# irfanfadhullah/unet_zoo

Measured on AMD Instinct MI355X. Metric: images/sec (fwd+bwd) at B=16 3x256x256, 1/2/4/8 MI355X, higher is better.
Workload: dtype bf16; 1 GPU; unet train step (zero_grad+fwd+BCE+bwd+clip+AdamW), B=16/GPU 3x256x256, random-init weights; global_batch=16, parallelism=dp1

## Files before the change

include/unetzoo_hip.h:

```cpp
#ifndef UNETZOO_HIP_H
#define UNETZOO_HIP_H

#include <stddef.h>
#include <stdint.h>

#ifdef __cplusplus
extern "C" {
#endif

#define UZ_ABI_VERSION 1

enum { UZ_F32 = 0, UZ_BF16 = 1 };

enum {
  UZ_OK = 0,
  UZ_EINVAL = -1,
  UZ_ENOTIMPL = -2
};

enum {
  UZ_TAPS_CONV = 0,
  UZ_TAPS_GATHER2X2 = 1,
  UZ_TAPS_CONV_UP2 = 2,
  UZ_TAPS_CONV_S2 = 3
// ... 10 lines not shown
int uz_build_ablate(void);
const char* uz_source_hash(void);
int uz_clock_probe(int iters, void* out_pairs, int workgroups, void* stream);
int uz_set_cu_reserve(int n);
int uz_get_cu_reserve(void);

typedef struct uz_conv_desc {
  int dtype;
  int N, H, W;
  int Hin, Win;
  int Cin, ldx;
  int Nout, ldy;
  int ntaps, taps_mode, dil;
  int store_mode, Co;
  int Hout, Wout;
} uz_conv_desc;

int uz_conv_igemm_grid_m(const uz_conv_desc* d);
int uz_conv_igemm_kernel_name(const uz_conv_desc* d, int with_workspace, char* buf, int cap);
int uz_conv_igemm(const uz_conv_desc* d, const void* x, const void* w_packed, const float* bias,
                  void* y, float* stats_partial, void* stream);
int uz_conv_igemm_res(const uz_conv_desc* d, const void* x, const void* w_packed, const float* bias,
                      const void* res, int ldres, void* y, void* stream);
int uz_conv_igemm_res_ws(const uz_conv_desc* d, const void* x, const void* w_packed, const float* bias,
                         const void* res, int ldres, void* y, void* workspace, void* stream);
long long uz_conv_igemm_workspace_bytes(const uz_conv_desc* d);
int uz_conv_igemm_ws_grid_m(const uz_conv_desc* d);
int uz_conv_igemm_ws(const uz_conv_desc* d, const void* x, const void* w_packed, const float* bias,
                     void* y, float* stats_partial, void* workspace, void* stream);
int uz_conv_igemm_bnred_supported(const uz_conv_desc* d);
int uz_conv_igemm_bnred(const uz_conv_desc* d, const void* x, const void* w_packed, void* y, const void* bn_y,
                        int ld_bny, const float* scale, const float* shift, const float* mean, const float* invstd,
                        float* partial, void* stream);

int uz_conv_igemm_xf_supported(const uz_conv_desc* d);
int uz_conv_igemm_xf(const uz_conv_desc* d, const void* x, const float* in_scale, const float* in_shift,
                     const void* w_packed, const float* bias, void* y, float* stats_partial, void* stream);

int uz_conv_igemm_bnact_supported(const uz_conv_desc* d);
int uz_conv_igemm_bnact(const uz_conv_desc* d, const void* x, const void* w_packed, const float* bias,
                        const float* out_scale, const float* out_shift, int relu, void* y, void* stream);

typedef struct uz_wgrad_desc {
  int dtype;
  int N, H, W;
  int Hr, Wr;
  int Ci, ldl;
  int Cj, ldr;
  int ntaps, taps_mode, dil;
} uz_wgrad_desc;

int uz_wgrad_split(const uz_wgrad_desc* d);
long long uz_wgrad_workspace_bytes(const uz_wgrad_desc* d);
int uz_wgrad(const uz_wgrad_desc* d, const void* L, const void* R, float* out, void* workspace,
             void* stream);
int uz_wgrad_kernel_name(const uz_wgrad_desc* d, char* buf, int cap);
int uz_wgrad_xf_supported(const uz_wgrad_desc* d);
int uz_wgrad_xf(const uz_wgrad_desc* d, const void* L, const void* R, const float* r_scale, const float* r_shift,
                float* out, void* workspace, void* stream, int phase);
int uz_wgrad_phase(const uz_wgrad_desc* d, const void* L, const void* R, float* out, void* workspace, void* stream,
                   int phase);
typedef struct {
  uz_wgrad_desc desc;
  const void* L;
  const void* R;
  float* out;
// ... 383 lines not shown
```

unet_zoo_amd/_lib.py:

```python
from __future__ import annotations

import ctypes
import os
from ctypes import POINTER, Structure, c_char_p, c_double, c_float, c_int, c_void_p

import torch

UZ_F32, UZ_BF16 = 0, 1
TAPS_CONV, TAPS_GATHER2X2, TAPS_CONV_UP2, TAPS_CONV_S2 = 0, 1, 2, 3
STORE_PLAIN, STORE_SHUFFLE2X2 = 0, 1
PACK_CONV_FWD, PACK_CONV_DGRAD, PACK_CONVT_FWD, PACK_CONVT_DGRAD, PACK_IM2COL, PACK_VEC_REPEAT = range(6)

LIB_NAME = "libunetzoo_hip.so"
LIB_PATH = os.environ.get("UNET_ZOO_AMD_LIB") or os.path.join(os.path.dirname(os.path.abspath(__file__)), LIB_NAME)

EXPORTS = (
    "uz_abi_version", "uz_last_error_string", "uz_build_ablate", "uz_source_hash", "uz_set_cu_reserve", "uz_get_cu_reserve", "uz_clock_probe", "uz_conv_igemm_grid_m", "uz_conv_igemm",
    "uz_wgrad_split", "uz_wgrad_workspace_bytes", "uz_wgrad", "uz_wgrad_kernel_name", "uz_wgrad_phase", "uz_wgrad_xf_supported", "uz_wgrad_xf", "uz_conv3x3_first_supported", "uz_conv3x3_first_rows", "uz_conv3x3_first_fwd",
    "uz_conv3x3_first_wgrad_workspace_bytes", "uz_conv3x3_first_wgrad", "uz_conv3x3_first_wgrad_bn", "uz_pack_weights", "uz_pack_weights_batched", "uz_pack_conv3x3_batched", "uz_im2col3x3_nchw", "uz_bn_finalize",
    "uz_bn_eval_scale", "uz_bn_relu_apply", "uz_bn_relu_bwd_workspace_bytes", "uz_bn_relu_bwd_reduce", "uz_bn_relu_bwd_apply",
    "uz_outconv_fwd", "uz_outconv_fwd_xf", "uz_outconv_bwd_workspace_bytes", "uz_outconv_bwd", "uz_outconv_bwd_rows", "uz_outconv_bwd_bnred", "uz_bn_relu_bwd_apply_head_supported", "uz_bn_relu_bwd_apply_head",
    "uz_colsum",
    "uz_attn_grid", "uz_attn_psi_fwd", "uz_attn_gate_fwd", "uz_attn_bwd_psi", "uz_attn_bwd_reduce",
    "uz_attn_bwd_apply", "uz_sum_rows", "uz_sum_rows_f32", "uz_sum2x2",
    "uz_bn_relu_add_apply", "uz_bn_relu_add_apply_fin", "uz_bn_relu_bwd_reduce_rows", "uz_bn_relu_bwd_apply_fin", "uz_bilinear_fwd", "uz_bilinear_bwd", "uz_resize_bilinear_fwd", "uz_resize_bilinear_bwd", "uz_resample2",
    "uz_pool_grad_combine",
    "uz_sideconv3x3_fwd", "uz_sideconv3x3_bwd_workspace_bytes", "uz_sideconv3x3_bwd",
    "uz_fuse1x1_fwd", "uz_fuse1x1_bwd_workspace_bytes", "uz_fuse1x1_bwd",
    "uz_conv_igemm_workspace_bytes", "uz_conv_igemm_ws_grid_m", "uz_conv_igemm_ws",
    "uz_conv_igemm_bnred_supported", "uz_conv_igemm_bnred", "uz_conv_igemm_xf_supported", "uz_conv_igemm_xf", "uz_conv_igemm_kernel_name", "uz_bn_bwd_finalize", "uz_profile_arm", "uz_profile_disarm",
    "uz_patchify", "uz_layernorm_fwd", "uz_layernorm_bwd_rows", "uz_layernorm_bwd", "uz_layernorm_act_bwd",
    "uz_ln_head_fwd", "uz_ln_head_bwd_workspace_bytes", "uz_ln_head_bwd", "uz_sum_rows_f32_ld",
    "uz_winattn_fwd", "uz_winattn_bwd_rows", "uz_winattn_bwd",
    "uz_colsum_workspace_bytes", "uz_colsum_ws", "uz_colstats_rows", "uz_colstats", "uz_cpb_fwd", "uz_cpb_bwd",
    "uz_cpb_fwd_batched", "uz_cpb_bwd_batched_workspace_bytes", "uz_cpb_bwd_batched",
    "uz_clip_adamw_workspace_bytes", "uz_clip_adamw",
    "uz_gelu_fwd", "uz_gelu_bwd", "uz_dwconv3x3", "uz_dwconv3x3_wgrad_rows", "uz_dwconv3x3_wgrad",
    "uz_space_to_depth", "uz_space_to_depth_crop", "uz_im2col_nchw", "uz_sra_fwd", "uz_sra_bwd_workspace_bytes", "uz_sra_bwd",
    "uz_bce_dice_workspace_bytes", "uz_bce_dice", "uz_colsum_batched_workspace_bytes", "uz_colsum_batched", "uz_sum_rows_f32_batched", "uz_conv_igemm_res", "uz_wgrad_multi_workspace_bytes", "uz_wgrad_multi", "uz_conv_igemm_res_ws",
    "uz_add_relu", "uz_relu_bwd", "uz_pil_resample_h_u8", "uz_pil_resample_v_f32",
    "uz_gemm_nt", "uz_softmax_fwd", "uz_softmax_bwd", "uz_adaptive_avgpool_fwd", "uz_adaptive_avgpool_bwd",
    "uz_rowdot_f32", "uz_cast_rows", "uz_wgrad_batched_workspace_bytes", "uz_wgrad_batched", "uz_wgrad_batched2",
    "uz_softmax_workspace_bytes", "uz_add_map", "uz_dropout", "uz_chanscale_relu", "uz_chanattn_probs_fwd", "uz_chanattn_probs_bwd",
    "uz_conv5x5_grid_m", "uz_conv5x5", "uz_wgrad5x5_workspace_bytes", "uz_wgrad5x5",
    "uz_bn_elu_apply", "uz_bn_elu_bwd_rows", "uz_bn_elu_bwd_reduce", "uz_bn_elu_bwd_apply",
    "uz_conv_igemm_bnact_supported", "uz_conv_igemm_bnact", "uz_conv3x3_first_fwd_bnact",
    "uz_region_loss_workspace_bytes", "uz_region_loss",
)


class ConvDesc(Structure):
    _fields_ = [(n, c_int) for n in (
        "dtype", "N", "H", "W", "Hin", "Win", "Cin", "ldx", "Nout", "ldy", "ntaps", "taps_mode",
        "dil", "store_mode", "Co", "Hout", "Wout")]


class WgradDesc(Structure):
    _fields_ = [(n, c_int) for n in (
        "dtype", "N", "H", "W", "Hr", "Wr", "Ci", "ldl", "Cj", "ldr", "ntaps", "taps_mode", "dil")]


class Conv5Desc(Structure):
    _fields_ = [(n, c_int) for n in ("dtype", "N", "H", "W", "Cin", "ldx", "Nout", "ldy", "ksize")]


class Wgrad5Desc(Structure):
    _fields_ = [(n, c_int) for n in ("dtype", "N", "H", "W", "Ci", "ldl", "Cj", "ldr", "ksize", "CiOut", "CjOut")]


class BnEluBwdDesc(Structure):
    _fields_ = [(n, c_int) for n in ("dtype", "N", "HW", "C", "ldx", "ldo", "ldg0", "ldg1", "ldg2", "lddx", "ldgres", "flags")]


class BnBwdDesc(Structure):
    _fields_ = [(n, c_int) for n in (
        "dtype", "N", "H", "W", "C", "ldy", "ldg0", "ldg1", "ldgp", "lddy", "pool_ceil")]


class LnDesc(Structure):
    _fields_ = [(n, c_int) for n in ("dtype", "N", "Ho", "Wo", "C", "ldx", "ldy", "ldr", "ldg", "lddx", "mode", "r")] \
        + [("eps", c_float), ("act", c_int)]


class WinAttnDesc(Structure):
    _fields_ = [(n, c_int) for n in ("dtype", "B", "H", "W", "C", "heads", "ws", "shift", "Nt", "ldq", "ldo")] \
        + [("scale", c_float)]

# ... 65 lines not shown
    global _lib
    if _lib is not None:
        return _lib
    if not os.path.exists(LIB_PATH):
        raise HipLibraryError(
            f"{LIB_PATH} not found: the HIP kernel library is not built. Run "
            "`python -c 'import __graft_entry__ as g; g.build()'` from the repo root. "
            "unet_zoo_amd has no CPU fallback.")
    lib = ctypes.CDLL(LIB_PATH)
    lib.uz_abi_version.restype = c_int
    lib.uz_last_error_string.restype = c_char_p
    lib.uz_source_hash.restype = c_char_p
    lib.uz_source_hash.argtypes = []
    vp, ip, fp = c_void_p, c_int, c_float
    lib.uz_set_cu_reserve.argtypes = [c_int]
    lib.uz_clock_probe.argtypes = [c_int, vp, c_int, vp]
    lib.uz_get_cu_reserve.argtypes = []
    lib.uz_conv_igemm_grid_m.argtypes = [POINTER(ConvDesc)]
    lib.uz_conv_igemm.argtypes = [POINTER(ConvDesc), vp, vp, vp, vp, vp, vp]
    lib.uz_conv_igemm_res.argtypes = [POINTER(ConvDesc), vp, vp, vp, vp, ip, vp, vp]
    lib.uz_conv_igemm_res_ws.argtypes = [POINTER(ConvDesc), vp, vp, vp, vp, ip, vp, vp, vp]
    lib.uz_conv_igemm_workspace_bytes.argtypes = [POINTER(ConvDesc)]
    lib.uz_conv_igemm_ws_grid_m.argtypes = [POINTER(ConvDesc)]
    lib.uz_conv_igemm_ws.argtypes = [POINTER(ConvDesc), vp, vp, vp, vp, vp, vp, vp]
    lib.uz_conv_igemm_bnred_supported.argtypes = [POINTER(ConvDesc)]
    lib.uz_conv_igemm_xf_supported.argtypes = [POINTER(ConvDesc)]
    lib.uz_conv_igemm_xf.argtypes = [POINTER(ConvDesc), vp, vp, vp, vp, vp, vp, vp, vp]
    lib.uz_conv_igemm_bnact_supported.argtypes = [POINTER(ConvDesc)]
    lib.uz_conv_igemm_bnact.argtypes = [POINTER(ConvDesc), vp, vp, vp, vp, vp, c_int, vp, vp]
    lib.uz_conv_igemm_kernel_name.argtypes = [POINTER(ConvDesc), c_int, c_char_p, c_int]
    lib.uz_profile_arm.argtypes = [vp, vp]
    lib.uz_profile_disarm.argtypes = []
    lib.uz_conv_igemm_bnred.argtypes = [POINTER(ConvDesc), vp, vp, vp, vp, c_int, vp, vp, vp, vp, vp, vp]
    lib.uz_bn_bwd_finalize.argtypes = [vp, c_int, c_int, vp, vp, vp, vp]
    lib.uz_patchify.argtypes = [ip, vp, ip, ip, ip, ip, ip, ip, vp, vp]
    lib.uz_layernorm_fwd.argtypes = [POINTER(LnDesc), vp, vp, vp, vp, vp, vp, vp, vp]
    lib.uz_layernorm_act_bwd.argtypes = [POINTER(LnDesc), vp, vp, vp, vp, vp, vp, vp, vp]
    lib.uz_layernorm_bwd_rows.argtypes = [POINTER(LnDesc)]
    lib.uz_layernorm_bwd.argtypes = [POINTER(LnDesc), vp, vp, vp, vp, vp, vp, vp, vp]
    lib.uz_ln_head_fwd.argtypes = [POINTER(LnDesc), vp, vp, vp, vp, vp, ip, vp, vp, vp]
    lib.uz_ln_head_bwd_workspace_bytes.argtypes = [POINTER(LnDesc), ip]
    lib.uz_ln_head_bwd.argtypes = [POINTER(LnDesc), vp, vp, vp, vp, ip, vp, vp, vp, vp, vp, vp, vp, vp, vp]
    lib.uz_sum_rows_f32_ld.argtypes = [vp, ip, ip, ip, vp, ip, vp, vp]
    lib.uz_winattn_fwd.argtypes = [POINTER(WinAttnDesc), vp, vp, vp, vp, vp, vp]
    lib.uz_winattn_bwd_rows.argtypes = [POINTER(WinAttnDesc)]
    lib.uz_winattn_bwd.argtypes = [POINTER(WinAttnDesc), vp, vp, vp, vp, vp, vp, ip, vp, ip, vp, vp]
    lib.uz_colstats_rows.argtypes = [ip, ip, ip]
    lib.uz_colstats.argtypes = [ip, vp, ip, ip, ip, vp, vp]
    lib.uz_cpb_fwd.argtypes = [vp, vp, vp, vp, vp, ip, ip, ip, vp, vp]
    lib.uz_cpb_bwd.argtypes = [vp, vp, vp, vp, vp, ip, ip, ip, vp, vp, vp, vp, vp]
    lib.uz_cpb_fwd_batched.argtypes = [vp, ip, vp]
    lib.uz_cpb_bwd_batched_workspace_bytes.argtypes = [vp, ip]
    lib.uz_cpb_bwd_batched.argtypes = [vp, ip, vp, vp]
    lib.uz_clip_adamw_workspace_bytes.argtypes = []
    lib.uz_clip_adamw.argtypes = [vp, vp, vp, vp, ctypes.c_longlong, fp, fp, fp, fp, fp, fp, vp, vp, vp]
    lib.uz_wgrad_split.argtypes = [POINTER(WgradDesc)]
    lib.uz_wgrad_workspace_bytes.argtypes = [POINTER(WgradDesc)]
    lib.uz_wgrad.argtypes = [POINTER(WgradDesc), vp, vp, vp, vp, vp]
    lib.uz_wgrad_kernel_name.argtypes = [POINTER(WgradDesc), c_char_p, c_int]
    lib.uz_wgrad_phase.argtypes = [POINTER(WgradDesc), vp, vp, vp, vp, vp, c_int]
    lib.uz_wgrad_xf_supported.argtypes = [POINTER(WgradDesc)]
    lib.uz_wgrad_xf.argtypes = [POINTER(WgradDesc), vp, vp, vp, vp, vp, vp, vp, c_int]
    lib.uz_conv3x3_first_supported.argtypes = [ip, ip, ip]
    lib.uz_conv3x3_first_rows.argtypes = [ip, ip, ip]
    lib.uz_conv3x3_first_fwd.argtypes = [ip, vp, ip, ip, ip, ip, vp, vp, ip, vp, ip, vp, vp]
    lib.uz_conv3x3_first_fwd_bnact.argtypes = [ip, vp, ip, ip, ip, ip, vp, vp, ip, vp, vp, ip, vp, ip, vp]
# ... 191 lines not shown
```

unet_zoo_amd/engine.py:

```python
from __future__ import annotations

import math
from typing import Callable, Dict, List, Optional, Sequence, Tuple

import torch
import torch.nn as nn

from . import _lib as L
from . import ops
from .ops import Act


def _round_up(a: int, b: int) -> int:
    return (a + b - 1) // b * b


class PackCache:

    def __init__(self):
        self.entries: Dict[tuple, tuple] = {}
        self._table: Optional[torch.Tensor] = None
        self._total = 0
        self._n = 0
        self._table_dtype = None
# ... 59 lines not shown
        begin = 0
        for i, (p, mode, kpad, dst) in enumerate(generic):
            if mode == L.PACK_VEC_REPEAT:
                arr[i] = L.PackItem(p.data_ptr(), dst.data_ptr(), begin, mode, p.numel(), 1, kpad, 0, 0)
                begin += dst.numel()
                continue
            d0, d1 = p.shape[0], p.shape[1]
            T = p.numel() // (d0 * d1)
            co, ci = (d0, d1) if mode in (L.PACK_CONV_FWD, L.PACK_CONV_DGRAD, L.PACK_IM2COL) else (d1, d0)
            arr[i] = L.PackItem(p.data_ptr(), dst.data_ptr(), begin, mode, co, ci, T, kpad, 0)
            begin += dst.numel()
        self._table = torch.frombuffer(bytearray(bytes(arr)), dtype=torch.uint8).to(dev)
        self._total, self._n, self._table_dtype = begin, len(generic), dtype

class ImageInput:

    __slots__ = ("nchw", "kpad", "dtype", "_patches", "N", "H", "W")

    def __init__(self, nchw: torch.Tensor, kpad: int, dtype: torch.dtype):
        self.nchw, self.kpad, self.dtype, self._patches = nchw, kpad, dtype, None
        self.N, _, self.H, self.W = nchw.shape

    def patches(self) -> Act:
        if self._patches is None:
            self._patches = ops.im2col3x3_nchw(self.nchw, self.kpad, self.dtype)
        return self._patches


class Engine:
    direct_first_conv = True
    defer_linear_wgrads = True
    fuse_bn_reduce = True
    fuse_bn_reduce_convt = True
    fold_bn_apply = True
    fold_bn_apply_head = True
    fold_head_grad = True
    fold_first_bn_bwd = True
    fuse_bn_finalize = False
    FIN_FLAGS = 4096
    reverse_element_passes = True
    fold_bn_eval = False

    def __init__(self, dtype: torch.dtype, device: torch.device, training: bool, record: bool,
                 grad_sink: Optional[Callable[[nn.Parameter, torch.Tensor], None]] = None,
                 pack_cache: Optional[PackCache] = None, grads_in_place: bool = False,
                 fold_bn_eval: Optional[bool] = None):
        if fold_bn_eval is not None:
            self.fold_bn_eval = bool(fold_bn_eval)
        self.folded_layers = 0
        self.unfolded_layers = 0
        self.dtype = dtype
        self.device = device
        self.training = training
        self.record = record
        self.tape: List[Callable[[], None]] = []
        self.param_grads: Dict[nn.Parameter, torch.Tensor] = {}
        self.grad_sink = grad_sink
        self.bk = 64 if dtype == torch.bfloat16 else 32
        self._bn_channels = 0
        self._sums: Optional[torch.Tensor] = None
        self._sums_used = 0
        self._cache = pack_cache if pack_cache is not None else PackCache()
        self.grads_in_place = grads_in_place
        self._heads: List[Tuple[Callable[..., None], int]] = []
        self.grad_log: List[Tuple[int, nn.Parameter]] = []
        self._pending_colsums: List[Tuple[int, nn.Parameter, Act]] = []
# ... 565 lines not shown
        return out

    def input_nhwc(self, x: torch.Tensor, cpad: int = 8) -> Act:
        L.require_cuda(x)
        N, C, H, W = x.shape
        a = self.new_act(N, H, W, _round_up(C, cpad), needs_grad=False)
        a.buf.zero_()
        a.buf.view(N, H, W, a.C)[..., :C].copy_(x.permute(0, 2, 3, 1))
        return a

    def act_to_logits(self, x: Act, K: int) -> torch.Tensor:
        assert K <= x.C
        logits = x.buf.view(x.N, x.H, x.W, x.ld)[..., x.off:x.off + K].permute(0, 3, 1, 2).float().contiguous()
        if self.record:
            def bwd(g_logits: torch.Tensor):
                g = self.new_act(x.N, x.H, x.W, x.C)
                g.buf.zero_()
                g.buf.view(x.N, x.H, x.W, x.C)[..., :K].copy_(g_logits.permute(0, 2, 3, 1))
                x.add_grad(g)

            self._heads.append((bwd, 1))
        return logits

    def conv_transpose2x2(self, x: Act, m: nn.ConvTranspose2d, out: Act, sole_reader: bool = False) -> Act:
        assert m.kernel_size == (2, 2) and m.stride == (2, 2) and m.in_channels == x.C
        Co = m.out_channels
        assert out.C == Co and out.H - 2 * x.H in (0, 1) and out.W - 2 * x.W in (0, 1)
        if (out.H, out.W) != (2 * x.H, 2 * x.W):
            v = out.buf.view(out.N, out.H, out.W, out.ld)[..., out.off:out.off + Co]
            v[:, 2 * x.H:, :, :] = 0
            v[:, :, 2 * x.W:, :] = 0
        wp = self._pack(m.weight, L.PACK_CONVT_FWD)
        bias4 = self._cache.get(m.bias, L.PACK_VEC_REPEAT, 4, self.dtype) if m.bias is not None else None
        ops.conv_igemm(x, wp, bias4, out, ntaps=1, store_mode=L.STORE_SHUFFLE2X2, nout=4 * Co, co=Co)

        if self.record:
            def bwd():
                g = self._sum_grads(out, 1)[0]
                if m.bias is not None:
                    cs = g.channel_sums(out=self._dst(m.bias))
                    self._give_grad(m.bias, cs if cs is not None else ops.colsum(g, out=self._dst(m.bias)))
                self._give_grad(m.weight, ops.wgrad(x, g, tuple(m.weight.shape), ntaps=4,
                                                    taps_mode=L.TAPS_GATHER2X2, out=self._dst(m.weight)))
                if x.needs_grad:
                    dx = self.new_act(x.N, x.H, x.W, x.C)
                    src = getattr(x, "bn_src", None) if (sole_reader and self.fuse_bn_reduce_convt) else None
                    part = ops.conv_igemm(g, self._pack(m.weight, L.PACK_CONVT_DGRAD), None, dx, ntaps=4,
                                          taps_mode=L.TAPS_GATHER2X2, bnred=src)
                    if src is not None and part is not None:
                        dx.bn_partials = part
                    x.add_grad(dx)

            self.tape.append(bwd)
        return out

    def _total_grad(self, a: Act) -> Optional[Act]:
        gs = list(a.grads)
        if not gs:
            return None
        while len(gs) > 1:
            g1, g0 = gs.pop(), gs.pop()
            tot = self.new_act(a.N, a.H, a.W, a.C)
            ops.pool_grad_combine(a, g0, g1, None, tot)
            gs.append(tot)
        return gs[0]

    def linear(self, x: Act, lin: nn.Linear, out: Optional[Act] = None, residual: Optional[Act] = None) -> Act:
        assert lin.in_features == x.C
        y = out if out is not None else self.new_act(x.N, x.H, x.W, lin.out_features)
        ops.conv_igemm(x, self._pack(lin.weight, L.PACK_CONV_FWD), lin.bias.detach() if lin.bias is not None else None,
                       y, ntaps=1, res=residual)
        if self.record:
            def bwd():
                g = self._total_grad(y)
                if g is None:
                    return
                if residual is not None and residual.needs_grad:
                    residual.add_grad(g)
                if lin.bias is not None:
                    self._bias_grad(lin.bias, g)
                self._linear_wgrad(lin.weight, g, x)
# ... 1151 lines not shown
```

unet_zoo_amd/ops.py:

```python
from __future__ import annotations

from ctypes import byref
from typing import List, Optional, Sequence

import math

import torch

from . import _lib as L


class Act:

    __slots__ = ("buf", "off", "C", "N", "H", "W", "grads", "parts", "rparts", "needs_grad", "colsums", "bn_src",
                 "bn_partials", "lazy")

    def __init__(self, buf: torch.Tensor, off: int, C: int, N: int, H: int, W: int,
                 needs_grad: bool = True):
        assert buf.dim() == 2 and buf.is_contiguous() and buf.shape[0] == N * H * W
        assert 0 <= off and off + C <= buf.shape[1]
        self.buf, self.off, self.C, self.N, self.H, self.W = buf, off, C, N, H, W
        self.grads: List["Act"] = []
        self.parts: Optional[Sequence["Act"]] = None
        self.rparts: Optional[Sequence[tuple]] = None
# ... 288 lines not shown
            L.check(lib.uz_conv_igemm_xf(byref(d), x.ptr(), xform[0].data_ptr(), xform[1].data_ptr(), w_packed.data_ptr(),
                                         _p(bias), y.ptr(), _p(stats), L.stream_ptr()), "uz_conv_igemm_xf")
        return stats
    if bnred is not None:
        assert bias is None and res is None and not want_stats
        bn_y, vec4 = bnred
        if not lib.uz_conv_igemm_bnred_supported(byref(d)) or (bn_y.P, bn_y.C) != (y.P, y.C):
            bnred = None
        else:
            gm = L.check_count(lib.uz_conv_igemm_grid_m(byref(d)), "uz_conv_igemm_grid_m")
            part = torch.empty((gm, 2, d.Nout), dtype=torch.float32, device=x.buf.device)
            with _Timed(kname + "_bnred", 2.0 * M * d.Nout * K, es * (x.P * x.C + 2 * M * d.Nout + d.Nout * K)):
                L.check(lib.uz_conv_igemm_bnred(byref(d), x.ptr(), w_packed.data_ptr(), y.ptr(), bn_y.ptr(), bn_y.ld,
                                                vec4[0].data_ptr(), vec4[1].data_ptr(), vec4[2].data_ptr(),
                                                vec4[3].data_ptr(), part.data_ptr(), L.stream_ptr()),
                        "uz_conv_igemm_bnred")
            return part
    if res is not None:
        assert (res.P, res.C) == (y.P, y.C) and res.dtype == y.dtype and not want_stats
        if kname.startswith("gemm_dma") and store_mode == L.STORE_PLAIN:
            with _Timed(kname, 2.0 * M * d.Nout * K, es * (x.P * x.C + 2 * M * d.Nout + d.Nout * K)):
                L.check(lib.uz_conv_igemm_res_ws(byref(d), x.ptr(), w_packed.data_ptr(), _p(bias), res.ptr(), res.ld, y.ptr(),
                                                 _p(ws), L.stream_ptr()), "uz_conv_igemm_res_ws")
            return None
    with _Timed(kname, 2.0 * M * d.Nout * K,
                        es * (x.P * x.C + M * d.Nout + d.Nout * K)):
        L.check(lib.uz_conv_igemm_ws(byref(d), x.ptr(), w_packed.data_ptr(), _p(bias), y.ptr(), _p(stats),
                                     _p(ws), L.stream_ptr()), "uz_conv_igemm_ws")
    if res is not None:
        add_acts(y, res, y)
    return stats


def _bnact_desc(x: Act, nout: int, ldy: int, ntaps: int, dil: int, taps_mode: int):
    H, W = (2 * x.H, 2 * x.W) if taps_mode == L.TAPS_CONV_UP2 else (x.H, x.W)
    return L.ConvDesc(L.dtype_code(x.dtype), x.N, H, W, x.H, x.W, x.C, x.ld, nout, ldy, ntaps, taps_mode, dil,
                      L.STORE_PLAIN, 0, 0, 0)


def conv_bnact_supported(x: Act, nout: int, ldy: int, *, ntaps: int, dil: int = 1, taps_mode: int = L.TAPS_CONV) -> bool:
    if taps_mode not in (L.TAPS_CONV, L.TAPS_CONV_UP2):
        return False
    d = _bnact_desc(x, nout, ldy, ntaps, dil, taps_mode)
    return bool(L.load().uz_conv_igemm_bnact_supported(byref(d)))


def conv_igemm_bnact(x: Act, w_packed: torch.Tensor, bias: Optional[torch.Tensor], scale: torch.Tensor, shift: torch.Tensor,
                     relu: bool, y: Act, *, ntaps: int, dil: int = 1, taps_mode: int = L.TAPS_CONV) -> None:
    L.require_cuda(x.buf, w_packed, y.buf, scale, shift)
    d = _bnact_desc(x, y.C, y.ld, ntaps, dil, taps_mode)
    assert w_packed.dtype == x.dtype and y.dtype == x.dtype and (y.N, y.H, y.W) == (d.N, d.H, d.W)
    assert w_packed.shape == (d.Nout, ntaps * x.C), (tuple(w_packed.shape), d.Nout, ntaps, x.C)
    assert scale.dtype == shift.dtype == torch.float32 and scale.numel() == shift.numel() == d.Nout
    assert scale.is_contiguous() and shift.is_contiguous()
    M, K, es = d.N * d.H * d.W, ntaps * x.C, x.buf.element_size()
    with _Timed(conv_kernel_name(d) + "_bnact", 2.0 * M * d.Nout * K, es * (x.P * x.C + M * d.Nout + d.Nout * K)):
        L.check(L.load().uz_conv_igemm_bnact(byref(d), x.ptr(), w_packed.data_ptr(), _p(bias), scale.data_ptr(),
                                             shift.data_ptr(), 1 if relu else 0, y.ptr(), L.stream_ptr()), "uz_conv_igemm_bnact")


def conv_first_fwd_bnact(x: torch.Tensor, w: torch.Tensor, bias: Optional[torch.Tensor], scale: torch.Tensor,
                         shift: torch.Tensor, relu: bool, y: Act) -> None:
    L.require_cuda(x, w, y.buf, scale, shift)
    assert x.dtype == torch.float32 and x.is_contiguous() and w.dtype == torch.float32 and w.is_contiguous()
    N, C, H, W = x.shape
    Cout = w.shape[0]
# ... 1072 lines not shown
```

Measured before the change: 2580 images/sec.

## Add warp-specialized streaming ConvTranspose2x2 kernels for forward and dgrad

Adds a dedicated HIP kernel for 2x2 stride-2 ConvTranspose forward and input-gradient. It uses producer waves that issue buffer-to-LDS loads for activations and weights, and MFMA consumer waves that keep each activation tile resident across all output-channel chunks. The kernel is persistent across tiles and stages output through LDS so stores are coalesced, with an optional fused BN-reduction variant for dgrad. The engine routes eligible shapes to it by default and falls back to the generic implicit-GEMM path otherwise. The new kernel only covers narrow shapes (Cin 128/256 forward, Cin 64 to 128 dgrad) and relies on hand-written waitcnt/barrier choreography, which could be fragile.

```diff
diff --git a/include/unetzoo_hip.h b/include/unetzoo_hip.h
--- a/include/unetzoo_hip.h
+++ b/include/unetzoo_hip.h
@@ -66,6 +66,19 @@
 int uz_conv_igemm_bnred(const uz_conv_desc* d, const void* x, const void* w_packed, void* y, const void* bn_y,
                         int ld_bny, const float* scale, const float* shift, const float* mean, const float* invstd,
                         float* partial, void* stream);
+
+typedef struct uz_convt_bnred {
+  const void* bn_y;
+  int ld_bny;
+  const float *scale, *shift, *mean, *invstd;
+  float* partial;
+} uz_convt_bnred;
+int uz_convt2x2_supported(const uz_conv_desc* d);
+int uz_convt2x2_grid_m(const uz_conv_desc* d);
+int uz_convt2x2_kernel_name(const uz_conv_desc* d, char* buf, int cap);
+int uz_convt2x2_fwd(const uz_conv_desc* d, const void* x, const void* w_packed, const float* bias, void* y, void* stream);
+int uz_convt2x2_dgrad(const uz_conv_desc* d, const void* g, const void* w_packed, void* dx, const uz_convt_bnred* br,
+                      void* stream);
 
 int uz_conv_igemm_xf_supported(const uz_conv_desc* d);
 int uz_conv_igemm_xf(const uz_conv_desc* d, const void* x, const float* in_scale, const float* in_shift,
diff --git a/unet_zoo_amd/_lib.py b/unet_zoo_amd/_lib.py
--- a/unet_zoo_amd/_lib.py
+++ b/unet_zoo_amd/_lib.py
@@ -28,6 +28,7 @@
     "uz_sideconv3x3_fwd", "uz_sideconv3x3_bwd_workspace_bytes", "uz_sideconv3x3_bwd",
     "uz_fuse1x1_fwd", "uz_fuse1x1_bwd_workspace_bytes", "uz_fuse1x1_bwd",
     "uz_conv_igemm_workspace_bytes", "uz_conv_igemm_ws_grid_m", "uz_conv_igemm_ws",
+    "uz_convt2x2_supported", "uz_convt2x2_grid_m", "uz_convt2x2_kernel_name", "uz_convt2x2_fwd", "uz_convt2x2_dgrad",
     "uz_conv_igemm_bnred_supported", "uz_conv_igemm_bnred", "uz_conv_igemm_xf_supported", "uz_conv_igemm_xf", "uz_conv_igemm_kernel_name", "uz_bn_bwd_finalize", "uz_profile_arm", "uz_profile_disarm",
     "uz_patchify", "uz_layernorm_fwd", "uz_layernorm_bwd_rows", "uz_layernorm_bwd", "uz_layernorm_act_bwd",
     "uz_ln_head_fwd", "uz_ln_head_bwd_workspace_bytes", "uz_ln_head_bwd", "uz_sum_rows_f32_ld",
@@ -53,6 +54,11 @@
     _fields_ = [(n, c_int) for n in (
         "dtype", "N", "H", "W", "Hin", "Win", "Cin", "ldx", "Nout", "ldy", "ntaps", "taps_mode",
         "dil", "store_mode", "Co", "Hout", "Wout")]
+
+
+class ConvtBnRed(Structure):
+    _fields_ = [("bn_y", c_void_p), ("ld_bny", c_int), ("scale", c_void_p), ("shift", c_void_p), ("mean", c_void_p),
+                ("invstd", c_void_p), ("partial", c_void_p)]
 
 
 class WgradDesc(Structure):
@@ -184,6 +190,11 @@
     lib.uz_profile_arm.argtypes = [vp, vp]
     lib.uz_profile_disarm.argtypes = []
     lib.uz_conv_igemm_bnred.argtypes = [POINTER(ConvDesc), vp, vp, vp, vp, c_int, vp, vp, vp, vp, vp, vp]
+    lib.uz_convt2x2_supported.argtypes = [POINTER(ConvDesc)]
+    lib.uz_convt2x2_grid_m.argtypes = [POINTER(ConvDesc)]
+    lib.uz_convt2x2_kernel_name.argtypes = [POINTER(ConvDesc), c_char_p, c_int]
+    lib.uz_convt2x2_fwd.argtypes = [POINTER(ConvDesc), vp, vp, vp, vp, vp]
+    lib.uz_convt2x2_dgrad.argtypes = [POINTER(ConvDesc), vp, vp, vp, POINTER(ConvtBnRed), vp]
     lib.uz_bn_bwd_finalize.argtypes = [vp, c_int, c_int, vp, vp, vp, vp]
     lib.uz_patchify.argtypes = [ip, vp, ip, ip, ip, ip, ip, ip, vp, vp]
     lib.uz_layernorm_fwd.argtypes = [POINTER(LnDesc), vp, vp, vp, vp, vp, vp, vp, vp]
diff --git a/unet_zoo_amd/csrc/uz_convt.hip b/unet_zoo_amd/csrc/uz_convt.hip
--- /dev/null
+++ b/unet_zoo_amd/csrc/uz_convt.hip
@@ -0,0 +1,455 @@
+#include "uz_common.h"
+#include <string.h>
+
+namespace {
+
+struct CArgs {
+  const void* x;
+  const void* w;
+  void* y;
+  const float* bias;
+  float* stats;
+  const void* bn_y;
+  const float *bn_scale, *bn_shift, *bn_mean, *bn_invstd;
+  int ld_bny;
+  unsigned xbytes, wbytes;
+  int M, H, W, Hin, Win, ldx, N, ldy, Co, Hout, Wout, tiles_m, nch;
+};
+
+typedef __attribute__((address_space(3))) void* lds_ptr_t;
+constexpr unsigned OOB = 0x80000000u;
+
+template <int N> __device__ __forceinline__ void wait_vmcnt() {
+  asm volatile("s_waitcnt vmcnt(%0)" ::"n"(N) : "memory");
+}
+__device__ __forceinline__ void wg_barrier() {
+  asm volatile("" ::: "memory");
+  __builtin_amdgcn_s_barrier();
+  asm volatile("" ::: "memory");
+}
+__device__ __forceinline__ void pin16(Vec16<bf16_t>& v) {
+  unsigned* r = reinterpret_cast<unsigned*>(&v);
+  asm volatile("" : "+v"(r[0]), "+v"(r[1]), "+v"(r[2]), "+v"(r[3]));
+}
+
+enum { CT_FWD = 0, CT_DGRAD = 1, CT_DGRAD_SUMS = 2 };
+
+constexpr int BM = 128, BN = 64;
+constexpr int NSA = 6, NSW = 4;
+constexpr int A_SLAB = BM * 128, W_STAGE = BN * 128;
+constexpr int RSC = BN * 2 + 16;
+constexpr int TAB_FLOATS = 2048;
+constexpr int W_OFF = NSA * A_SLAB, C_OFF = W_OFF + NSW * W_STAGE, T_OFF = C_OFF + BM * RSC, LDS_BYTES = T_OFF + TAB_FLOATS * 4;
+constexpr int NCONS = 512;
+constexpr int APW = 8, WPW = 4;
+
+template <int KS, int MODE, int NCH>
+__global__ __launch_bounds__(768) void convt2x2_kernel(const CArgs a) {
+  static_assert(LDS_BYTES <= 160 * 1024, "LDS");
+  static_assert(MODE != CT_DGRAD_SUMS || NCH > 0, "the sums form needs a compile-time chunk count");
+  static_assert(MODE == CT_FWD || KS % 4 == 0, "four taps");
+  __shared__ __attribute__((aligned(16))) char smem[LDS_BYTES];
+  const int tid = threadIdx.x, lane = tid & 63;
+  const int wave = __builtin_amdgcn_readfirstlane(tid >> 6);
+  const int nch = NCH > 0 ? NCH : a.nch;
+  const int grid = gridDim.x;
+  const int ntl = (a.tiles_m - (int)blockIdx.x + grid - 1) / grid;
+  const int HW = a.H * a.W;
+
+  if (wave >= 10) {
+    const int la = wave - 10;
+    const __amdgpu_buffer_rsrc_t xr = __builtin_amdgcn_make_buffer_rsrc(const_cast<void*>(a.x), 0, a.xbytes, 0x00020000);
+    const int total = ntl * KS;
+    unsigned abase[APW];
+    int coff[APW];
+    auto issue = [&](int i) {
+      const int tl = i / KS, k = i - tl * KS;
+      if (k == 0) {
+        const int m0 = ((int)blockIdx.x + tl * grid) * BM;
+#pragma unroll
+        for (int p = 0; p < APW; ++p) {
+          const int row = (la + 2 * p) * 8 + (lane >> 3);
+          const int m = m0 + row;
+          coff[p] = ((lane & 7) ^ ((row >> 1) & 7)) * 16;
+          unsigned pix;
+          if (MODE == CT_FWD) {
+            pix = (unsigned)m;
+          } else {
+            const int mm = m < a.M ? m : 0;
+            const int img = mm / HW, rem = mm - img * HW;
+            const int h = rem / a.W, w = rem - h * a.W;
+            pix = (unsigned)((img * a.Hin + 2 * h) * a.Win + 2 * w);
+          }
+          abase[p] = m < a.M ? pix * (unsigned)(a.ldx * 2) : OOB;
+        }
+      }
+      unsigned soff;
+      if (MODE == CT_FWD) {
+        soff = (unsigned)k * 128u;
+      } else {
+        constexpr int SPT = KS / 4;
+        const int tap = k / SPT, cb = k - tap * SPT;
+        soff = (unsigned)((tap >> 1) * a.Win + (tap & 1)) * (unsigned)(a.ldx * 2) + (unsigned)cb * 128u;
+      }
+      char* dst = smem + (i % NSA) * A_SLAB;
+#pragma unroll
+      for (int p = 0; p < APW; ++p) {
+        const unsigned off = abase[p] != OOB ? abase[p] + soff + (unsigned)coff[p] : OOB;
+        __builtin_amdgcn_raw_ptr_buffer_load_lds(xr, (lds_ptr_t)(dst + (la + 2 * p) * 1024), 16, off, 0, 0, 0);
+      }
+    };
+    int iss = 0;
+    for (; iss < NSA && iss < total; ++iss) issue(iss);
+    wg_barrier();
+    for (int tl = 0; tl < ntl; ++tl)
+      for (int c = 0; c < nch; ++c) {
+#pragma unroll 1
+        for (int k = 0; k < KS; ++k) {
+          if (c == 0) {
+            switch (iss - 1 - (tl * KS + k)) {
+              case 0: wait_vmcnt<0>(); break;
+              case 1: wait_vmcnt<APW>(); break;
+              case 2: wait_vmcnt<2 * APW>(); break;
+              case 3: wait_vmcnt<3 * APW>(); break;
+              case 4: wait_vmcnt<4 * APW>(); break;
+              default: wait_vmcnt<5 * APW>(); break;
+            }
+          }
+          wg_barrier();
+          const int retired = tl * KS + (c == nch - 1 ? k : 0);
+          for (; iss < retired + NSA && iss < total; ++iss) issue(iss);
+        }
+        wg_barrier();
+      }
+    if (MODE == CT_DGRAD_SUMS) {
+      wg_barrier();
+      wg_barrier();
+    }
+    return;
+  }
+
+  if (wave >= 8) {
+    const int lw = wave - 8;
+    const __amdgpu_buffer_rsrc_t wr = __builtin_amdgcn_make_buffer_rsrc(const_cast<void*>(a.w), 0, a.wbytes, 0x00020000);
+    const int total = ntl * nch * KS;
+    const unsigned ldw = (unsigned)KS * 128u;
+    unsigned wrow[WPW];
+#pragma unroll
+    for (int p = 0; p < WPW; ++p) {
+      const int row = (lw + 2 * p) * 8 + (lane >> 3);
+      wrow[p] = (unsigned)row * ldw + (unsigned)(((lane & 7) ^ ((row >> 1) & 7)) * 16);
+    }
+    int ic = 0, ik = 0, ig = 0;
+    auto issue = [&]() {
+      char* dst = smem + W_OFF + (ig % NSW) * W_STAGE;
+      const unsigned base = (unsigned)ic * (BN * ldw) + (unsigned)ik * 128u;
+#pragma unroll
+      for (int p = 0; p < WPW; ++p)
+        __builtin_amdgcn_raw_ptr_buffer_load_lds(wr, (lds_ptr_t)(dst + (lw + 2 * p) * 1024), 16, base + wrow[p], 0, 0, 0);
+      ++ig;
+      if (++ik == KS) {
+        ik = 0;
+        if (++ic == nch) ic = 0;
+      }
+    };
+    for (int i = 0; i < NSW - 1 && i < total; ++i) issue();
+    wg_barrier();
+    int g = 0;
+    for (int tl = 0; tl < ntl; ++tl)
+      for (int c = 0; c < nch; ++c) {
+#pragma unroll 1
+        for (int k = 0; k < KS; ++k, ++g) {
+          if (g + 2 < total) wait_vmcnt<2 * WPW>();
+          else if (g + 1 < total) wait_vmcnt<WPW>();
+          else wait_vmcnt<0>();
+          wg_barrier();
+          if (g + NSW - 1 < total) issue();
+        }
+        wg_barrier();
+      }
+    if (MODE == CT_DGRAD_SUMS) {
+      wg_barrier();
+      wg_barrier();
+    }
+    return;
+  }
+
+  const int l31 = lane & 31, lh = lane >> 5;
+  const int wm = wave >> 1, wn = wave & 1;
+  const int arow = wm * 32 + l31, brow = wn * 32 + l31;
+  const int a_frag = arow * 128, a_sw = (arow >> 1) & 7;
+  const int b_frag = brow * 128, b_sw = (brow >> 1) & 7;
+  bf16_t* __restrict__ yg = static_cast<bf16_t*>(a.y);
+  char* sC = smem + C_OFF;
+  constexpr int CPR = BN * 2 / 16, RPP = NCONS / CPR, NPASS = BM / RPP;
+  const int cc = tid % CPR, r0 = tid / CPR;
+  constexpr int NSUM = MODE == CT_DGRAD_SUMS ? NCH : 1;
+  float sq1[NSUM][8], sq2[NSUM][8];
+#pragma unroll
+  for (int c = 0; c < NSUM; ++c)
+#pragma unroll
+    for (int e = 0; e < 8; ++e) sq1[c][e] = sq2[c][e] = 0.f;
+
+  float* tab = reinterpret_cast<float*>(smem + T_OFF);
+  if (MODE == CT_FWD) {
+    for (int i = tid; i < a.N; i += NCONS) tab[i] = a.bias != nullptr ? a.bias[i] : 0.f;
+  } else if (MODE == CT_DGRAD_SUMS) {
+    for (int i = tid; i < a.N; i += NCONS) {
+      tab[i] = a.bn_scale[i];
+      tab[a.N + i] = a.bn_shift[i];
+    }
+  }
+  asm volatile("s_waitcnt lgkmcnt(0)" ::: "memory");
+  wg_barrier();
+
+  int g = 0;
+  for (int tl = 0; tl < ntl; ++tl) {
+    const int m0 = ((int)blockIdx.x + tl * grid) * BM;
+    long long orow[NPASS];
+#pragma unroll
+    for (int p = 0; p < NPASS; ++p) {
+      const int m = m0 + r0 + p * RPP;
+      if (m >= a.M) {
+        orow[p] = -1;
+      } else if (MODE == CT_FWD) {
+        const int img = m / HW, rem = m - img * HW;
+        const int h = rem / a.W, w = rem - h * a.W;
+        orow[p] = ((long long)img * a.Hout + 2 * h) * a.Wout + 2 * w;
+      } else {
+        orow[p] = m;
+      }
+    }
+    for (int c = 0; c < nch; ++c) {
+      const int n0 = c * BN;
+      Vec16<bf16_t> yb[NPASS];
+      if constexpr (MODE == CT_DGRAD_SUMS) {
+        const bf16_t* by = static_cast<const bf16_t*>(a.bn_y);
+#pragma unroll
+        for (int p = 0; p < NPASS; ++p)
+          yb[p] = ld16(by + (orow[p] >= 0 ? (size_t)orow[p] * a.ld_bny + n0 + cc * 8 : 0));
+      }
+      float bq[16];
+#pragma unroll
+      for (int r = 0; r < 16; ++r)
+        bq[r] = MODE == CT_FWD ? tab[n0 + wn * 32 + (r & 3) + 8 * (r >> 2) + 4 * lh] : 0.f;
+      f32x16 acc;
+#pragma unroll
+      for (int r = 0; r < 16; ++r) acc[r] = 0.f;
+#pragma unroll
+      for (int k = 0; k < KS; ++k, ++g) {
+        asm volatile("s_waitcnt lgkmcnt(0)" ::: "memory");
+        wg_barrier();
+        const char* sA = smem + ((tl * KS + k) % NSA) * A_SLAB;
+        const char* sW = smem + W_OFF + (g % NSW) * W_STAGE;
+#pragma unroll
+        for (int q = 0; q < 4; ++q) {
+          const int lc = 2 * q + lh;
+          const bf16x8 af = *reinterpret_cast<const bf16x8*>(sA + a_frag + ((lc ^ a_sw) << 4));
+          const bf16x8 bf = *reinterpret_cast<const bf16x8*>(sW + b_frag + ((lc ^ b_sw) << 4));
+          acc = __builtin_amdgcn_mfma_f32_32x32x16_bf16(bf, af, acc, 0, 0, 0);
+        }
+      }
+      {
+        char* rowp = sC + arow * RSC;
+#pragma unroll
+        for (int q = 0; q < 4; ++q) {
+          bf16x4 pk;
+#pragma unroll
+          for (int e = 0; e < 4; ++e)
+            pk[e] = (bf16_t)(MODE == CT_DGRAD_SUMS ? acc[4 * q + e] : acc[4 * q + e] + bq[4 * q + e]);
+          *reinterpret_cast<bf16x4*>(rowp + (wn * 32 + 8 * q + 4 * lh) * 2) = pk;
+        }
+      }
+      asm volatile("s_waitcnt lgkmcnt(0)" ::: "memory");
+      wg_barrier();
+      Vec16<bf16_t> vb[NPASS];
+#pragma unroll
+      for (int p = 0; p < NPASS; ++p)
+        vb[p] = *reinterpret_cast<const Vec16<bf16_t>*>(sC + (r0 + p * RPP) * RSC + cc * 16);
+      int cot = n0 + cc * 8;
+      long long shift = 0;
+      if (MODE == CT_FWD) {
+        const int ab = cot / a.Co;
+        cot -= ab * a.Co;
+        shift = (long long)(ab >> 1) * a.Wout + (ab & 1);
+      }
+      float bsc[8], bsh[8];
+      if constexpr (MODE == CT_DGRAD_SUMS) {
+#pragma unroll
+        for (int p = 0; p < NPASS; ++p) pin16(yb[p]);
+#pragma unroll
+        for (int e = 0; e < 8; e += 4) {
+          *reinterpret_cast<f32x4*>(&bsc[e]) = *reinterpret_cast<const f32x4*>(tab + cot + e);
+          *reinterpret_cast<f32x4*>(&bsh[e]) = *reinterpret_cast<const f32x4*>(tab + a.N + cot + e);
+        }
+      }
+#pragma unroll
+      for (int p = 0; p < NPASS; ++p) {
+        if (orow[p] >= 0) {
+          st16(yg + (size_t)(orow[p] + shift) * a.ldy + cot, vb[p]);
+          if constexpr (MODE == CT_DGRAD_SUMS) {
+            const int cs = c;
+#pragma unroll
+            for (int e = 0; e < 8; ++e) {
+              const float yv = (float)yb[p].v[e];
+              const float dz = fmaf(yv, bsc[e], bsh[e]) > 0.f ? (float)vb[p].v[e] : 0.f;
+              sq1[cs][e] += dz;
+              sq2[cs][e] += dz * yv;
+            }
+          }
+        }
+      }
+    }
+  }
+
+  if constexpr (MODE == CT_DGRAD_SUMS) {
+    wg_barrier();
+    float* red = reinterpret_cast<float*>(smem);
+#pragma unroll
+    for (int c = 0; c < NCH; ++c)
+#pragma unroll
+      for (int e = 0; e < 8; ++e) {
+        red[((tid * NCH + c) * 2 + 0) * 8 + e] = sq1[c][e];
+        red[((tid * NCH + c) * 2 + 1) * 8 + e] = sq2[c][e];
+      }
+    asm volatile("s_waitcnt lgkmcnt(0)" ::: "memory");
+    wg_barrier();
+    for (int i = tid; i < 2 * NCH * BN; i += NCONS) {
+      const int which = i / (NCH * BN), n = i - which * (NCH * BN);
+      const int c = n / BN, ch = n - c * BN;
+      const int ck = ch / 8, e = ch - ck * 8;
+      float t = 0.f, t0 = 0.f;
+      for (int k = ck; k < NCONS; k += CPR) {
+        t += red[((k * NCH + c) * 2 + which) * 8 + e];
+        t0 += red[((k * NCH + c) * 2 + 0) * 8 + e];
+      }
+      if (which == 1) t = a.bn_invstd[n] * (t - a.bn_mean[n] * t0);
+      a.stats[((size_t)blockIdx.x * 2 + which) * a.N + n] = t;
+    }
+  }
+}
+
+int convt_form(const uz_conv_desc* d) {
+  if (d == nullptr || d->dtype != UZ_BF16) return 0;
+  if (d->N <= 0 || d->H <= 0 || d->W <= 0) return 0;
+  const long long M = (long long)d->N * d->H * d->W, pin = (long long)d->N * d->Hin * d->Win;
+  if (M >= (1LL << 31) - BM || pin >= (1LL << 31)) return 0;
+  if (d->ldx % 8 != 0 || d->ldy % 8 != 0 || d->ldx < d->Cin) return 0;
+  const long long xbytes = (pin - 1) * d->ldx * 2 + (long long)d->Cin * 2;
+  const long long wbytes = (long long)d->Nout * d->ntaps * d->Cin * 2;
+  if (xbytes >= (1LL << 31) || wbytes >= (1LL << 31)) return 0;
+  if (d->taps_mode == UZ_TAPS_CONV && d->ntaps == 1 && d->store_mode == UZ_STORE_SHUFFLE2X2) {
+    if (d->Hin != d->H || d->Win != d->W) return 0;
+    if ((d->Cin != 128 && d->Cin != 256) || d->Co <= 0 || d->Co % 64 != 0 || d->Nout != 4 * d->Co || d->Nout > TAB_FLOATS || d->ldy < d->Co) return 0;
+    const int Ho = d->Hout ? d->Hout : 2 * d->H, Wo = d->Wout ? d->Wout : 2 * d->W;
+    if ((Ho != 2 * d->H && Ho != 2 * d->H + 1) || (Wo != 2 * d->W && Wo != 2 * d->W + 1)) return 0;
+    return 1;
+  }
+  if (d->taps_mode == UZ_TAPS_GATHER2X2 && d->ntaps == 4 && d->store_mode == UZ_STORE_PLAIN) {
+    if ((d->Hin != 2 * d->H && d->Hin != 2 * d->H + 1) || (d->Win != 2 * d->W && d->Win != 2 * d->W + 1)) return 0;
+    if (d->Cin != 64 || d->Nout != 128 || d->ldy < d->Nout) return 0;
+    return 2;
+  }
+  return 0;
+}
+
+int convt_grid(const uz_conv_desc* d) {
+  const long long tiles = ((long long)d->N * d->H * d->W + BM - 1) / BM;
+  return (int)(tiles < UZ_NUM_CU_HW ? tiles : UZ_NUM_CU_HW);
+}
+
+void fill_args(const uz_conv_desc* d, CArgs* a) {
+  memset(a, 0, sizeof(*a));
+  const long long pin = (long long)d->N * d->Hin * d->Win;
+  a->xbytes = (unsigned)((pin - 1) * d->ldx * 2 + (long long)d->Cin * 2);
+  a->wbytes = (unsigned)((long long)d->Nout * d->ntaps * d->Cin * 2);
+  a->M = d->N * d->H * d->W;
+  a->H = d->H;
+  a->W = d->W;
+  a->Hin = d->Hin;
+  a->Win = d->Win;
+  a->ldx = d->ldx;
+  a->N = d->Nout;
+  a->ldy = d->ldy;
+  a->Co = d->Co > 0 ? d->Co : d->Nout;
+  a->Hout = d->Hout ? d->Hout : 2 * d->H;
+  a->Wout = d->Wout ? d->Wout : 2 * d->W;
+  a->tiles_m = (a->M + BM - 1) / BM;
+  a->nch = d->Nout / BN;
+}
+
+}
+
+extern "C" int uz_convt2x2_supported(const uz_conv_desc* d) { return convt_form(d) != 0 ? 1 : 0; }
+
+extern "C" int uz_convt2x2_grid_m(const uz_conv_desc* d) {
+  UZ_REQUIRE(convt_form(d) != 0, "uz_convt2x2_grid_m: the descriptor is not one of the streaming ConvTranspose forms "
+             "(ask uz_convt2x2_supported)");
+  return convt_grid(d);
+}
+
+extern "C" int uz_convt2x2_kernel_name(const uz_conv_desc* d, char* buf, int cap) {
+  const int form = convt_form(d);
+  UZ_REQUIRE(form != 0, "uz_convt2x2_kernel_name: the descriptor is not one of the streaming ConvTranspose forms");
+  UZ_REQUIRE(buf != nullptr && cap > 0, "uz_convt2x2_kernel_name: no buffer");
+  const char* name = form == 1 ? "convt2x2_fwd_bf16" : "convt2x2_dgrad_bf16";
+  snprintf(buf, (size_t)cap, "%s", name);
+  return (int)strlen(name);
+}
+
+extern "C" int uz_convt2x2_fwd(const uz_conv_desc* d, const void* x, const void* w_packed, const float* bias, void* y,
+                               void* stream) {
+  if (convt_form(d) != 1) {
+    uz_set_error("uz_convt2x2_fwd: bf16 ConvTranspose2d k2 s2 forward with Cin = 128 or 256 and Co a multiple of 64, tensors below "
+                 "2 GiB (ask uz_convt2x2_supported)");
+    return UZ_ENOTIMPL;
+  }
+  UZ_REQUIRE(x && w_packed && y, "uz_convt2x2_fwd: null pointer");
+  UZ_REQUIRE((((uintptr_t)x | (uintptr_t)w_packed | (uintptr_t)y) & 15) == 0, "uz_convt2x2_fwd: x / w / y must be 16-byte aligned");
+  CArgs a;
+  fill_args(d, &a);
+  a.x = x;
+  a.w = w_packed;
+  a.y = y;
+  a.bias = bias;
+  hipStream_t s = static_cast<hipStream_t>(stream);
+  if (d->Cin == 128) hipLaunchKernelGGL((convt2x2_kernel<2, CT_FWD, 0>), dim3(convt_grid(d)), dim3(768), 0, s, a);
+  else hipLaunchKernelGGL((convt2x2_kernel<4, CT_FWD, 0>), dim3(convt_grid(d)), dim3(768), 0, s, a);
+  UZ_LAUNCH_CHECK("uz_convt2x2_fwd");
+  return UZ_OK;
+}
+
+extern "C" int uz_convt2x2_dgrad(const uz_conv_desc* d, const void* g, const void* w_packed, void* dx,
+                                 const uz_convt_bnred* br, void* stream) {
+  if (convt_form(d) != 2) {
+    uz_set_error("uz_convt2x2_dgrad: bf16 ConvTranspose2d k2 s2 input gradient with Co = 64 and Cin = 128, tensors below "
+                 "2 GiB (ask uz_convt2x2_supported)");
+    return UZ_ENOTIMPL;
+  }
+  UZ_REQUIRE(g && w_packed && dx, "uz_convt2x2_dgrad: null pointer");
+  UZ_REQUIRE((((uintptr_t)g | (uintptr_t)w_packed | (uintptr_t)dx) & 15) == 0, "uz_convt2x2_dgrad: g / w / dx must be 16-byte aligned");
+  CArgs a;
+  fill_args(d, &a);
+  a.x = g;
+  a.w = w_packed;
+  a.y = dx;
+  hipStream_t s = static_cast<hipStream_t>(stream);
+  if (br != nullptr) {
+    UZ_REQUIRE(br->bn_y && br->scale && br->shift && br->mean && br->invstd && br->partial, "uz_convt2x2_dgrad: null pointer in the sums argument");
+    UZ_REQUIRE(((uintptr_t)br->bn_y & 15) == 0 && ((uintptr_t)br->scale & 15) == 0 && ((uintptr_t)br->shift & 15) == 0,
+               "uz_convt2x2_dgrad: bn_y / scale / shift must be 16-byte aligned");
+    UZ_REQUIRE(br->ld_bny >= d->Nout && br->ld_bny % 8 == 0, "uz_convt2x2_dgrad: bad ld_bny %d", br->ld_bny);
+    a.bn_y = br->bn_y;
+    a.ld_bny = br->ld_bny;
+    a.bn_scale = br->scale;
+    a.bn_shift = br->shift;
+    a.bn_mean = br->mean;
+    a.bn_invstd = br->invstd;
+    a.stats = br->partial;
+    hipLaunchKernelGGL((convt2x2_kernel<4, CT_DGRAD_SUMS, 2>), dim3(convt_grid(d)), dim3(768), 0, s, a);
+  } else {
+    hipLaunchKernelGGL((convt2x2_kernel<4, CT_DGRAD, 2>), dim3(convt_grid(d)), dim3(768), 0, s, a);
+  }
+  UZ_LAUNCH_CHECK("uz_convt2x2_dgrad");
+  return UZ_OK;
+}
diff --git a/unet_zoo_amd/engine.py b/unet_zoo_amd/engine.py
--- a/unet_zoo_amd/engine.py
+++ b/unet_zoo_amd/engine.py
@@ -115,6 +115,8 @@
     defer_linear_wgrads = True
     fuse_bn_reduce = True
     fuse_bn_reduce_convt = True
+    stream_convt_fwd = True
+    stream_convt_dgrad = True
     fold_bn_apply = True
     fold_bn_apply_head = True
     fold_head_grad = True
@@ -746,7 +748,10 @@
             v[:, :, 2 * x.W:, :] = 0
         wp = self._pack(m.weight, L.PACK_CONVT_FWD)
         bias4 = self._cache.get(m.bias, L.PACK_VEC_REPEAT, 4, self.dtype) if m.bias is not None else None
-        ops.conv_igemm(x, wp, bias4, out, ntaps=1, store_mode=L.STORE_SHUFFLE2X2, nout=4 * Co, co=Co)
+        if self.stream_convt_fwd and ops.convt2x2_supported(ops.convt_fwd_desc(x, out, Co)):
+            ops.convt2x2_fwd(x, wp, bias4, out, Co)
+        else:
+            ops.conv_igemm(x, wp, bias4, out, ntaps=1, store_mode=L.STORE_SHUFFLE2X2, nout=4 * Co, co=Co)
 
         if self.record:
             def bwd():
@@ -759,8 +764,11 @@
                 if x.needs_grad:
                     dx = self.new_act(x.N, x.H, x.W, x.C)
                     src = getattr(x, "bn_src", None) if (sole_reader and self.fuse_bn_reduce_convt) else None
-                    part = ops.conv_igemm(g, self._pack(m.weight, L.PACK_CONVT_DGRAD), None, dx, ntaps=4,
-                                          taps_mode=L.TAPS_GATHER2X2, bnred=src)
+                    if self.stream_convt_dgrad and ops.convt2x2_supported(ops.convt_dgrad_desc(g, dx)):
+                        part = ops.convt2x2_dgrad(g, self._pack(m.weight, L.PACK_CONVT_DGRAD), dx, bnred=src)
+                    else:
+                        part = ops.conv_igemm(g, self._pack(m.weight, L.PACK_CONVT_DGRAD), None, dx, ntaps=4,
+                                              taps_mode=L.TAPS_GATHER2X2, bnred=src)
                     if src is not None and part is not None:
                         dx.bn_partials = part
                     x.add_grad(dx)
diff --git a/unet_zoo_amd/ops.py b/unet_zoo_amd/ops.py
--- a/unet_zoo_amd/ops.py
+++ b/unet_zoo_amd/ops.py
@@ -344,6 +344,62 @@
     return stats
 
 
+def convt_fwd_desc(x: Act, y: Act, co: int):
+    return L.ConvDesc(L.dtype_code(x.dtype), x.N, x.H, x.W, x.H, x.W, x.C, x.ld, 4 * co, y.ld, 1, L.TAPS_CONV, 1,
+                      L.STORE_SHUFFLE2X2, co, y.H, y.W)
+
+
+def convt_dgrad_desc(g: Act, dx: Act):
+    return L.ConvDesc(L.dtype_code(g.dtype), g.N, g.H // 2, g.W // 2, g.H, g.W, g.C, g.ld, dx.C, dx.ld, 4, L.TAPS_GATHER2X2, 1,
+                      L.STORE_PLAIN, 0, 0, 0)
+
+
+def convt2x2_supported(d) -> bool:
+    return bool(L.load().uz_convt2x2_supported(byref(d)))
+
+
+def convt2x2_grid_m(d) -> int:
+    return L.check_count(L.load().uz_convt2x2_grid_m(byref(d)), "uz_convt2x2_grid_m")
+
+
+def convt2x2_kernel_name(d) -> str:
+    import ctypes
+    buf = ctypes.create_string_buffer(96)
+    L.check_count(L.load().uz_convt2x2_kernel_name(byref(d), buf, 96), "uz_convt2x2_kernel_name")
+    return buf.value.decode()
+
+
+def convt2x2_fwd(x: Act, w_packed: torch.Tensor, bias4: Optional[torch.Tensor], y: Act, co: int) -> None:
+    L.require_cuda(x.buf, w_packed, y.buf)
+    d = convt_fwd_desc(x, y, co)
+    assert w_packed.dtype == x.dtype == y.dtype and w_packed.shape == (4 * co, x.C)
+    M, es = x.P, x.buf.element_size()
+    with _Timed(convt2x2_kernel_name(d), 2.0 * M * d.Nout * x.C, es * (M * x.C + M * d.Nout + d.Nout * x.C)):
+        L.check(L.load().uz_convt2x2_fwd(byref(d), x.ptr(), w_packed.data_ptr(), _p(bias4), y.ptr(), L.stream_ptr()),
+                "uz_convt2x2_fwd")
+
+
+def convt2x2_dgrad(g: Act, w_packed: torch.Tensor, dx: Act, bnred: Optional[tuple] = None) -> Optional[torch.Tensor]:
+    L.require_cuda(g.buf, w_packed, dx.buf)
+    d = convt_dgrad_desc(g, dx)
+    assert w_packed.dtype == g.dtype == dx.dtype and w_packed.shape == (dx.C, 4 * g.C)
+    M, K, es = dx.P, 4 * g.C, g.buf.element_size()
+    kname = convt2x2_kernel_name(d)
+    if bnred is not None and (bnred[0].P, bnred[0].C) != (dx.P, dx.C):
+        bnred = None
+    br, part = None, None
+    if bnred is not None:
+        bn_y, vec4 = bnred
+        part = torch.empty((convt2x2_grid_m(d), 2, d.Nout), dtype=torch.float32, device=g.buf.device)
+        br = L.ConvtBnRed(bn_y.ptr(), bn_y.ld, vec4[0].data_ptr(), vec4[1].data_ptr(), vec4[2].data_ptr(), vec4[3].data_ptr(),
+                          part.data_ptr())
+    with _Timed(kname + ("_bnred" if br is not None else ""), 2.0 * M * d.Nout * K,
+                es * (g.P * g.C + (2 if br is not None else 1) * M * d.Nout + d.Nout * K)):
+        L.check(L.load().uz_convt2x2_dgrad(byref(d), g.ptr(), w_packed.data_ptr(), dx.ptr(), byref(br) if br is not None else None,
+                                           L.stream_ptr()), "uz_convt2x2_dgrad")
+    return part
+
+
 def _bnact_desc(x: Act, nout: int, ldy: int, ntaps: int, dil: int, taps_mode: int):
     H, W = (2 * x.H, 2 * x.W) if taps_mode == L.TAPS_CONV_UP2 else (x.H, x.W)
     return L.ConvDesc(L.dtype_code(x.dtype), x.N, H, W, x.H, x.W, x.C, x.ld, nout, ldy, ntaps, taps_mode, dil,
```

Measured after the change: 2590 images/sec, median of 3. About the same (+0.4%).
